# vpc-ccg/circminer

Measured on AMD Instinct MI355X. Metric: paired reads/sec (whole node), hg38 k=20, 2x150 bp; circ_report bit-exact, higher is better.
Workload: dtype int32/u8 (chain scores f64)

## Files before the change

circminer_amd/csrc/cm_hot.hip:

```cpp
#include <chrono>
#include <hip/hip_runtime.h>
#include <rocprim/device/device_radix_sort.hpp>

#include <algorithm>
#include <atomic>
#include <cstdarg>
#include <cstdio>
#include <cstdlib>
#include <cstring>
#include <string>
#include <functional>
#include <thread>
#include <vector>

#include "circminer_hot.h"
#include "cm_core.h"
#include "cm_aos.h"
#include "cm_index_build.h"

using cmc::Core;
using cmc::KCore;

namespace {

constexpr int MAX_SLOTS = 16;
constexpr uint32_t TILE_PAIRS = 1u << 20;
constexpr uint32_t TILE_PAIRS_MAX = 1u << 21;
constexpr int BLK = 256;
constexpr int BLK_CHAIN = 64;
#include "cm_dp_engine.h"

enum ProfClass { PC_NONE = -1, PC_SEED = 0, PC_CHAIN = 1, PC_PAIR = 2, PC_SCAN = 3, PC_HEAVY = 4, PC_ORDER = 5, PC_CHAIN_HEAVY = 6, PC_PREFETCH = 7, PC_COUNT = 8 };
enum Counter {
    CN_PROBES = 0 , CN_PAIR_ROUNDS = 3, CN_RERUN = 4 ,
    CN_FALL = 5, CN_FALL_2ND = 6,
    CN_CD_LANE = 8, CN_CD_PHASE = 13, CN_CD_WAVE = 16, CN_CD_EVENTS = 20, CN_CD_LEVELS = 21, CN_CD_PROBLEMS = 22, CN_CD_PASSES = 23, CN_CD_CELLS = 24,
    CN_HP_ATTEMPT = 8, CN_HP_STRIDE = 8, CN_HP_UNPAIRED = 24, CN_HP_CHAINS = 25, CN_HP_SEQ_TASKS = 26, CN_HP_EARLY = 27, CN_HP_EARLY_FIRST = 28,
    CN_WORDS = 32
};
static_assert(CN_CD_CELLS < CN_WORDS && CN_HP_EARLY_FIRST < CN_WORDS && CN_HP_ATTEMPT + CN_HP_STRIDE + 5 < CN_HP_UNPAIRED, "d_counters has CN_WORDS words");
enum Pin {
    PIN_COLLECT_N = 0, PIN_COLLECT_ERR = 1,
    PIN_DEV_ERR = 0,
    PIN_POOL_ERR = 2,
    PIN_HEAVY_LOAD = 4,
    PIN_CELLS = 8,
    PIN_RERUN_N = 12, PIN_FALL_N = 14,
    PIN_WORDS = 16
};
constexpr size_t PIN_BYTES = PIN_WORDS * sizeof(unsigned long long);
static_assert(PIN_BYTES == 128 && PIN_FALL_N + 1 < PIN_WORDS && PIN_CELLS + 3 < PIN_RERUN_N, "the landing zone has 16 words");
struct ReadsDev {
    const uint8_t *seq1, *seq2;
    const uint64_t *off1, *off2;
};

__global__ void __launch_bounds__(BLK) k_seed(KCore kc, ReadsDev rd, const uint8_t *active, uint64_t pair0, uint32_t n_tile, int S,
                                              uint32_t *sstart, uint32_t *scnt, uint32_t *sraw, unsigned long long *counters) {
    const Core c = cmc::to_core(kc);
    __shared__ unsigned int sh[3];
    if (threadIdx.x < 3) sh[threadIdx.x] = 0;
    __syncthreads();
    const uint64_t q = (uint64_t)blockIdx.x * BLK + threadIdx.x;
    const uint64_t total = (uint64_t)n_tile * 4u * (uint64_t)S;
    if (q < total) {
        const uint32_t s = (uint32_t)(q % (uint64_t)S);
        const uint64_t r = q / (uint64_t)S;
        const int orient = (int)(r & 1u), mate = (int)((r >> 1) & 1u);
        const uint64_t p = pair0 + (r >> 2);
        uint32_t st = 0, cn = 0, rw = 0;
        if (active[p]) {
            const uint64_t o0 = mate ? rd.off2[p] : rd.off1[p], o1 = mate ? rd.off2[p + 1] : rd.off1[p + 1];
            const int len = (int)(o1 - o0);
            const int k = c.P.kmer;
            if ((int)(s + 1) * k <= len) {
                const cmc::Read R{(cmc::g_u8)((mate ? rd.seq2 : rd.seq1) + o0), len, orient};
                const cmc::Probe pr = cmc::seed_probe(c, R.view(), (int)s * k);
                st = pr.start;
                rw = pr.raw;
                cn = (pr.raw > (uint32_t)c.P.seed_lim) ? 0u : pr.raw;
                atomicAdd(&sh[0], 1u);
                atomicAdd(&sh[1], pr.touches);
                atomicAdd(&sh[2], cn);
            }
        }
        sstart[q] = st;
        scnt[q] = cn;
        sraw[q] = rw;
    }
    __syncthreads();
    if (threadIdx.x < 3 && sh[threadIdx.x]) atomicAdd(&counters[CN_PROBES + threadIdx.x], (unsigned long long)sh[threadIdx.x]);
}

constexpr int SCAN_T = 256;
constexpr int SCAN_ELEMS = 1024;
__global__ void __launch_bounds__(SCAN_T) k_scan_a(const uint32_t *scnt, int S, uint32_t n, unsigned long long *out, unsigned long long *bsum,
                                                   unsigned int *bmax) {
    __shared__ unsigned long long sh[SCAN_T];
    __shared__ unsigned int shmax;
    const uint32_t base = blockIdx.x * SCAN_ELEMS;
    unsigned long long run = 0;
    unsigned int my_max = 0;
    if (threadIdx.x == 0) shmax = 0;
#pragma unroll
    for (int k = 0; k < SCAN_ELEMS / SCAN_T; ++k) {
        const uint32_t r = base + k * SCAN_T + threadIdx.x;
        uint32_t c = 0;
        if (r < n)
            for (int s = 0; s < S; ++s) c += scnt[(uint64_t)r * S + s];
        my_max = c > my_max ? c : my_max;
        sh[threadIdx.x] = c;
        __syncthreads();
        for (int d = 1; d < SCAN_T; d <<= 1) {
            const unsigned long long x = (threadIdx.x >= (unsigned)d) ? sh[threadIdx.x - d] : 0ull;
            __syncthreads();
            sh[threadIdx.x] += x;
            __syncthreads();
        }
        if (r < n) out[r] = run + sh[threadIdx.x] - c;
        run += sh[SCAN_T - 1];
        __syncthreads();
    }
    atomicMax(&shmax, my_max);
    __syncthreads();
    if (threadIdx.x == 0) {
        bsum[blockIdx.x] = run;
        bmax[blockIdx.x] = shmax;
    }
}
template <class T, bool WITH_MAX>
__global__ void __launch_bounds__(1024) k_scan_mid(T *bsum, uint32_t nb, T *total, const unsigned int *bmax) {
    __shared__ T part[1024];
    __shared__ unsigned int gmax;
    const uint32_t t = threadIdx.x;
    const uint32_t chunk = (nb + 1023u) / 1024u;
    const uint32_t a = t * chunk, b = (a + chunk < nb) ? a + chunk : nb;
    T s = 0;
    unsigned int m = 0;
    if (WITH_MAX && t == 0) gmax = 0;
    if constexpr (WITH_MAX) __syncthreads();
    for (uint32_t i = a; i < b; ++i) {
        s += bsum[i];
        if constexpr (WITH_MAX) m = bmax[i] > m ? bmax[i] : m;
    }
    if constexpr (WITH_MAX) atomicMax(&gmax, m);
    part[t] = s;
    __syncthreads();
    for (uint32_t d = 1; d < 1024; d <<= 1) {
        const T v = (t >= d) ? part[t - d] : (T)0;
        __syncthreads();
        part[t] += v;
        __syncthreads();
    }
    T run = t ? part[t - 1] : (T)0;
    for (uint32_t i = a; i < b; ++i) {
        const T x = bsum[i];
        bsum[i] = run;
        run += x;
    }
    if (WITH_MAX && t == 1023) {
        total[0] = part[1023];
        total[1] = gmax;
    }
}
__global__ void __launch_bounds__(SCAN_T) k_scan_c(unsigned long long *out, const unsigned long long *bsum, uint32_t n) {
    const uint32_t i = blockIdx.x * SCAN_T + threadIdx.x;
    if (i < n) out[i] += bsum[i / SCAN_ELEMS];
}

__device__ inline int pack_resid(int left, int right) {
    left = left < 0 ? 0 : (left > 255 ? 255 : left);
    right = right < 0 ? 0 : (right > 255 ? 255 : right);
    return left | (right << 8);
}
#ifndef CM_CHAIN_WAVES
#define CM_CHAIN_WAVES 5
#endif
__global__ void __launch_bounds__(BLK_CHAIN, CM_CHAIN_WAVES) k_chain(KCore kc, ReadsDev rd, const uint8_t *active, uint64_t pair0, uint32_t r0, uint32_t r1, int S,
                                                     const uint32_t *sstart, const uint32_t *scnt, const uint32_t *sraw,
                                                     const unsigned long long *celloff, unsigned long long cellbase, double *dp_score,
                                                     int32_t *dp_prev, uint8_t *pool, unsigned long long pool_bytes,
                                                     unsigned long long *pool_cursor, cm_chain *chains, int32_t *nchain, int32_t *high, int *err,
                                                     uint16_t *resid, const uint32_t *perm, const unsigned int *perm_lo, const unsigned int *perm_hi) {
    uint32_t r = r0 + blockIdx.x * BLK_CHAIN + threadIdx.x;
    if (perm) {
        r += *perm_lo;
        if (r >= *perm_hi) return;
        r = perm[r];
    } else if (r >= r1) return;
// ... 2 lines not shown
    int n = 0, hh = 0, rs = 0;
    if (active[p]) {
        const int mate = (int)((r >> 1) & 1u);
        const uint64_t o0 = mate ? rd.off2[p] : rd.off1[p], o1 = mate ? rd.off2[p + 1] : rd.off1[p + 1];
        const int len = (int)(o1 - o0);
        uint32_t st[cmc::MAX_SEEDS], cn[cmc::MAX_SEEDS];
        for (int s = 0; s < S; ++s) {
            st[s] = sstart[(uint64_t)r * S + s];
            cn[s] = scnt[(uint64_t)r * S + s];
            if (sraw[(uint64_t)r * S + s] > 0 && cn[s] == 0) ++hh;
        }
        cmc::ChainWork w;
        w.dp_score = (CM_G double *)(dp_score + (celloff[r] - cellbase));
        w.dp_prev = (CM_G int32_t *)(dp_prev + (celloff[r] - cellbase));
        w.pool = (CM_G uint8_t *)pool;
        w.pool_bytes = pool_bytes;
        w.pool_cursor = (CM_G unsigned long long *)pool_cursor;
        w.err = (cmc::g_err)err;
        n = cmc::chain_kbest(c, len, S, st, cn, w, (CM_G cm_chain *)(chains + (uint64_t)r * CM_BESTCHAINLIM));
        if (n > 0) {
            const cm_chain &b = chains[(uint64_t)r * CM_BESTCHAINLIM];
            rs = pack_resid(b.qpos[0], len - (b.qpos[b.chain_len - 1] + c.P.kmer));
        }
    }
    nchain[r] = n;
    high[r] = hh;
    resid[r] = (uint16_t)rs;
}

struct RetryArgs {
    uint32_t *pair_err;
    uint32_t *list;
    unsigned int *count;
    cmc::MemoSpill *spill;
    int spill_cap;
    int first;
};

template <bool FIRST>
__device__ __forceinline__ void pair_kernel(const KCore &kc, const ReadsDev &rd, uint64_t pair0, uint32_t n_tile, const cm_chain *chains, const int32_t *nchain,
                                            const int32_t *high, cm_mapped_read *state, uint8_t *active, int32_t *cat, int is_last,
                                            int *err, unsigned long long *counters, int str_cap, unsigned long long *lane_clk,
                                            const uint32_t *perm, const unsigned int *n_light, unsigned int *next_chunk,
                                            const RetryArgs &ra) {
    const unsigned long long clk0 = lane_clk ? wall_clock64() : 0ull;
    extern __shared__ uint32_t lds_words[];
#if defined(CM_DIAG)
    __shared__ unsigned long long tick_w[65];
    cmc::Tick tick;
    for (int i = 0; i < 32; ++i) tick.acc[i] = 0;
    tick.last = wall_clock64();
    tick.w = (CM_L unsigned long long *)tick_w;
    tick.wave_on = 1;
    for (int i = threadIdx.x; i < 65; i += BLK_PAIR) tick_w[i] = i == 0 ? tick.last : 0ull;
    __syncthreads();
    cmc::DpMem sm = lane_dp_mem((CM_S uint8_t *)lds_words, threadIdx.x, str_cap, (cmc::g_err)err, &tick);
#else
    cmc::DpMem sm = lane_dp_mem((CM_S uint8_t *)lds_words, threadIdx.x, str_cap, (cmc::g_err)err);
#endif
    if (ra.spill) {
        sm.spill = (cmc::g_spill)(ra.spill + ((size_t)blockIdx.x * BLK_PAIR + threadIdx.x) * (size_t)ra.spill_cap);
        sm.spill_cap = ra.spill_cap;
    }
    const Core c = cmc::to_core(kc);
    const uint32_t n_l = *n_light;
    auto take = [&]() { return (uint32_t)__shfl((int)(threadIdx.x == 0 ? atomicAdd(next_chunk, 1u) : 0u), 0); };
    for (uint32_t chunk = take(); (uint64_t)chunk * BLK_PAIR < n_l; chunk = take()) {
    const uint32_t slot = chunk * BLK_PAIR + threadIdx.x;
    if (slot >= n_l) continue;
    const unsigned long long it0 = lane_clk ? wall_clock64() : 0ull;
    const uint32_t t = perm[slot];
    const uint64_t p = pair0 + t;
    const uint64_t a0 = rd.off1[p], a1 = rd.off1[p + 1], b0 = rd.off2[p], b1 = rd.off2[p + 1];
    cmc::ChainSet sets[4];
    int hh[4];
    for (int x = 0; x < 4; ++x) {
        const uint64_t r = (uint64_t)t * 4 + x;
        sets[x].ch = (cmc::g_chain)(chains + r * CM_BESTCHAINLIM);
        sets[x].n = nchain[r];
        hh[x] = high[r];
    }
    cm_mapped_read mr = state[p];
#if defined(CM_AB_GLOBAL_ERR)
    int *perr = err;
#else
    int *perr = FIRST ? (int *)(ra.pair_err + t) : err;
    sm.err = (cmc::g_err)perr;
#endif
    const int st = cmc::process_read(c, sm, (cmc::g_u8)(rd.seq1 + a0), (int)(a1 - a0), (cmc::g_u8)(rd.seq2 + b0), (int)(b1 - b0), sets, hh, mr, (cmc::g_err)perr);
    bool keep = true;
    if (FIRST) {
        if (__hip_atomic_load(ra.pair_err + t, __ATOMIC_RELAXED, __HIP_MEMORY_SCOPE_AGENT) != 0u) {
            ra.list[atomicAdd(ra.count, 1u)] = t;
            active[pair0 + t] = 1;
            keep = false;
        }
    } else ra.pair_err[t] = 0u;
    if (keep) {
        uint8_t act = 1;
        cmc::finish_round(c, st, is_last, (int)(a1 - a0), (int)(b1 - b0), mr, act);
        state[p] = mr;
        active[p] = act;
        cat[p] = st;
    }
    {
        const unsigned long long m = __ballot(1), mk = __ballot(keep);
        if ((threadIdx.x & 63) == (unsigned)__ffsll((long long)m) - 1 && mk) {
            atomicAdd(&counters[CN_PAIR_ROUNDS], (unsigned long long)__popcll(mk));
            if (!FIRST) atomicAdd(&counters[CN_RERUN], (unsigned long long)__popcll(mk));
        }
    }
#if defined(CM_DIAG)
    CM_TICK(sm, 13);
    if (lane_clk) {
        for (int i = 0; i < 15; ++i) lane_clk[p * 16 + i] = tick.acc[i];
        lane_clk[p * 16 + 15] = wall_clock64() - clk0;
        const unsigned long long m = __ballot(1);
        if ((threadIdx.x & 63) == (unsigned)__ffsll((long long)m) - 1) {
            unsigned long long *wr = lane_clk + (unsigned long long)n_tile * 16 + (unsigned long long)blockIdx.x * 64;
            for (int i = 0; i < 64; ++i) wr[i] = tick_w[1 + i];
        }
    }
#else
    if (lane_clk) lane_clk[slot] = ((wall_clock64() - it0) & 0xFFFFFFFFull) | ((unsigned long long)t << 32);
#endif
    }
}


__global__ void __launch_bounds__(BLK_PAIR, CM_PAIR_WAVES) k_pair(KCore kc, ReadsDev rd, uint64_t pair0, uint32_t n_tile, const cm_chain *chains, const int32_t *nchain,
                                                   const int32_t *high, cm_mapped_read *state, uint8_t *active, int32_t *cat, int is_last,
                                                   int *err, unsigned long long *counters, int str_cap, unsigned long long *lane_clk,
                                                   const uint32_t *perm, const unsigned int *n_light, unsigned int *next_chunk,
                                                   RetryArgs ra) {
    pair_kernel<true>(kc, rd, pair0, n_tile, chains, nchain, high, state, active, cat, is_last, err, counters, str_cap, lane_clk, perm, n_light, next_chunk, ra);
}
__global__ void __launch_bounds__(BLK_PAIR, CM_PAIR_WAVES) k_pair_rerun(KCore kc, ReadsDev rd, uint64_t pair0, uint32_t n_tile, const cm_chain *chains,
                                                         const int32_t *nchain, const int32_t *high, cm_mapped_read *state, uint8_t *active, int32_t *cat,
                                                         int is_last, int *err, unsigned long long *counters, int str_cap,
                                                         unsigned long long *lane_clk, const uint32_t *perm, const unsigned int *n_light,
                                                         unsigned int *next_chunk, RetryArgs ra) {
    pair_kernel<false>(kc, rd, pair0, n_tile, chains, nchain, high, state, active, cat, is_last, err, counters, str_cap, lane_clk, perm, n_light, next_chunk, ra);
}

template <class T> __device__ inline T wave_excl_scan(T v, int lane, T &total) {
    T x = v;
    for (int o = 1; o < 64; o <<= 1) {
        const T y = __shfl_up(x, o);
        if (lane >= o) x += y;
    }
    total = __shfl(x, 63);
    return x - v;
}
struct HeavyChainCtx {
#if defined(CM_CHAIN_DIAG)
    unsigned long long *tk;
#endif
    const Core *c;
    CM_L const uint32_t *LP;
    CM_L const uint32_t *NB;
    CM_L const uint32_t *IM;
    const uint32_t *base, *cnt;
    int kc, seq_len;
    CM_G double *dps;
    CM_G int32_t *dpp;
};
__device__ inline uint32_t heavy_im_word(uint32_t base_s, uint32_t s) { return 2u * ((base_s >> 6) + s); }
__host__ __device__ inline uint32_t heavy_im_words(uint32_t ncell, uint32_t kc) { return 2u * ((ncell >> 6) + kc + 1u); }
__device__ inline uint32_t heavy_cell(const HeavyChainCtx &h, int ii, uint32_t i, CM_G cmc::Event *ev, double &out_score, int32_t &out_prev,
                                     double &e0, double &e1) {
    const Core &c = *h.c;
    const int kmer = c.P.kmer;
    const uint32_t read_remain = (uint32_t)(h.seq_len - ii * kmer - kmer);
    const int32_t cur_info = (int32_t)h.LP[h.base[ii] + i];
    const uint32_t seg_start = (uint32_t)cur_info, seg_end = (uint32_t)cur_info + kmer - 1;
    uint32_t max_lpos_lim = cmc::MAXUB, max_exon_end = 0;
    int ol = -1;
    double my_score = (double)kmer;
    int32_t my_prev = -1;
    uint32_t n = 0;
    const uint32_t cell = h.base[ii] + i;
    const bool near = (h.NB[cell >> 5] >> (cell & 31)) & 1u;
    uint2 parked = make_uint2(0u, 0u);
    int parked_ol = -1;
    if (near) {
        parked = *(CM_G const uint2 *)(h.dps + cell);
        parked_ol = h.dpp[cell];
    }
#if defined(CM_CHAIN_DIAG)
    if (!ev) h.tk[3] += 1;
#define CD_T0 const unsigned long long cd_t = wall_clock64()
#define CD_ADD(k) h.tk[k] += wall_clock64() - cd_t
#else
#define CD_T0
#define CD_ADD(k)
#endif
    for (int jj = ii + 1; jj < h.kc; ++jj) {
        const uint32_t pcn = h.cnt[jj];
        if (pcn == 0) continue;
        CM_L const uint32_t *pp = h.LP + h.base[jj];
        CM_L const uint32_t *im = h.IM + heavy_im_word(h.base[jj], (uint32_t)jj);
        uint32_t lo = 0, hi = pcn;
        {
            CD_T0;
            while (lo < hi) {
                const uint32_t mid = (lo + hi) >> 1;
                if ((int32_t)pp[mid] <= cur_info) lo = mid + 1;
                else hi = mid;
            }
            CD_ADD(0);
        }
        if (lo >= pcn) continue;
        if (cur_info + c.P.max_intron < (int32_t)pp[lo]) continue;
        if (max_lpos_lim == cmc::MAXUB) {
            CD_T0;
            if (near) {
                max_lpos_lim = parked.x;
                max_exon_end = parked.y;
                ol = parked_ol;
            } else {
                max_exon_end = 0;
                ol = -1;
                max_lpos_lim = seg_start + read_remain + (uint32_t)c.P.max_ed;
            }
            CD_ADD(1);
        }
        const int distr = (jj - ii) * kmer - kmer;
        CD_T0;
        for (uint32_t j = lo; j < pcn && pp[j] <= max_lpos_lim; ++j) {
#if defined(CM_CHAIN_DIAG)
            if (!ev) h.tk[4] += 1;
#endif
            const uint32_t pinfo = pp[j];
            int genome_dist, distt, trans_dist;
            if (max_exon_end == 0 || (pinfo + kmer - 1) <= max_exon_end) genome_dist = (int)(pinfo - seg_end - 1);
            else genome_dist = cmc::INF_I;
            if (cmc::cabs(genome_dist - distr) <= c.P.max_ed) distt = genome_dist;
            else if (cmc::check_junction(c, seg_start, pinfo, ol, kmer, distr, trans_dist)) distt = trans_dist;
            else continue;
            const int maxd = distr < distt ? distt : distr, mind = distr < distt ? distr : distt;
            const double beta = 0.1 * (double)(maxd - mind);
            const double alpha = 2e4 * (double)kmer;
            const double prev_score = ((im[j >> 5] >> (j & 31)) & 1u) ? h.dps[h.base[jj] + j] : (double)kmer;
            const double t1 = prev_score + alpha;
            const double temp_score = t1 - beta;
            if (temp_score > my_score) {
                my_score = temp_score;
                my_prev = (int32_t)(((uint32_t)jj << 16) | j);
                if (ev) {
                    ev[n].score = temp_score;
                    ev[n].cell = ((uint32_t)ii << 16) | i;
                }
                if (n == 0) e0 = temp_score;
                else if (n == 1) e1 = temp_score;
                ++n;
            }
        }
        CD_ADD(2);
    }
    out_score = my_score;
    out_prev = my_prev;
    return n;
}

struct HeavyBackTrack {
    uint32_t base[cmc::MAX_SEEDS + 1];
    uint32_t cand[CM_BESTCHAINLIM + 2];
    uint16_t cidx[CM_BESTCHAINLIM][CM_MAX_CHAIN_FRAGS];
    uint8_t cbl[CM_BESTCHAINLIM][CM_MAX_CHAIN_FRAGS];
    uint8_t clen[CM_BESTCHAINLIM + 2];
    uint8_t emit[CM_BESTCHAINLIM + 2];
    uint32_t rep[CM_BESTCHAINLIM * (CM_MAX_CHAIN_FRAGS - 1)];
};

#ifndef CM_CHEAVY_WAVES
#define CM_CHEAVY_WAVES 3
#endif
__global__ void __launch_bounds__(64, CM_CHEAVY_WAVES) k_chain_heavy(KCore kc_, ReadsDev rd, uint64_t pair0, int S, const uint32_t *sstart, const uint32_t *scnt,
                                                    const unsigned long long *celloff, double *dp_score, int32_t *dp_prev, uint8_t *pool,
                                                    unsigned long long pool_bytes, unsigned long long *pool_cursor, cm_chain *chains, int32_t *nchain,
                                                    int *err, uint16_t *resid, const uint32_t *perm, const unsigned int *n_perm, unsigned int *next_problem,
                                                    unsigned long long *counters) {
    extern __shared__ uint32_t lds_words[];
    CM_L uint32_t *LP = (CM_L uint32_t *)lds_words;
    __shared__ HeavyBackTrack BT;
    const int lane = threadIdx.x;
    const Core c = cmc::to_core(kc_);
    const int kmer = c.P.kmer;
    const uint32_t max_best = (uint32_t)c.P.max_chain_len;
    const unsigned int n_heavy = *n_perm;
    auto take = [&]() { return (unsigned int)__shfl((int)(lane == 0 ? atomicAdd(next_problem, 1u) : 0u), 0); };
    for (unsigned int hidx = take(); hidx < n_heavy; hidx = take()) {
        const uint32_t r = perm[hidx];
        const uint64_t p = pair0 + (r >> 2);
        const int mate = (int)((r >> 1) & 1u);
        const int len = (int)(mate ? rd.off2[p + 1] - rd.off2[p] : rd.off1[p + 1] - rd.off1[p]);
#if defined(CM_CHAIN_DIAG)
        const unsigned long long dg0 = wall_clock64();
#endif
        uint32_t st[cmc::MAX_SEEDS], cn[cmc::MAX_SEEDS], base[cmc::MAX_SEEDS + 1];
        int kc = S;
        for (int s = 0; s < S; ++s) {
            st[s] = sstart[(uint64_t)r * S + s];
            cn[s] = scnt[(uint64_t)r * S + s];
        }
        while (kc >= 1 && cn[kc - 1] == 0) --kc;
        base[0] = 0;
        for (int s = 0; s < kc; ++s) base[s + 1] = base[s] + cn[s];
        const uint32_t ncell = base[kc];
        CM_G double *dps = (CM_G double *)(dp_score + celloff[r]);
        CM_G int32_t *dpp = (CM_G int32_t *)(dp_prev + celloff[r]);
        CM_L uint32_t *NB = LP + ncell;
        CM_L uint16_t *Q = (CM_L uint16_t *)(NB + 2 * ((ncell + 63) >> 6));
        CM_L uint32_t *IM = (CM_L uint32_t *)(Q + 320);
        const bool by_entry = c.entry_near != nullptr;
        for (int s = 0; s < kc; ++s)
            for (uint32_t i = lane; i < cn[s]; i += 64) {
                const uint32_t e = st[s] + i;
                uint32_t v = c.X.pos[e];
                if (by_entry && s < kc - 1) v |= (uint32_t)((c.entry_near[e >> 6] >> (e & 63)) & 1ull) << 31;
                LP[base[s] + i] = v;
            }
        for (uint32_t x = lane; x < heavy_im_words(ncell, (uint32_t)kc); x += 64) IM[x] = 0u;
        __threadfence_block();
        __syncthreads();
        {
            const uint32_t n_pre = kc >= 1 ? base[kc - 1] : 0u;
            const unsigned long long lt = (1ull << lane) - 1ull;
            uint32_t qn = 0;
            auto look_up = [&](uint32_t cnt) {
                if ((uint32_t)lane < cnt) {
                    const uint32_t x = Q[lane];
                    int ii = 0;
                    for (int s = 1; s < kc; ++s) ii += x >= base[s] ? 1 : 0;
                    const uint32_t read_remain = (uint32_t)(len - ii * kmer - kmer);
                    uint32_t mx = 0;
                    int ol = -1;
                    const uint32_t lim = cmc::upper_bound_lookup(c, LP[x], (uint32_t)kmer, read_remain, mx, ol);
                    *(CM_G uint2 *)(dps + x) = make_uint2(lim, mx);
                    dpp[x] = ol;
                }
            };
            for (uint32_t x0 = 0; x0 < n_pre; x0 += 256) {
                bool nr[4];
#pragma unroll
                for (int u = 0; u < 4; ++u) {
                    const uint32_t x = x0 + 64 * u + lane;
                    if (by_entry) {
                        nr[u] = x < n_pre && (LP[x] >> 31);
                        if (nr[u]) LP[x] &= 0x7fffffffu;
                    } else nr[u] = x < n_pre && cmc::bit_at(c.A.near_border_bits, c.A.n_bits, LP[x]);
                }
#pragma unroll
                for (int u = 0; u < 4; ++u) {
                    const uint32_t xb = x0 + 64 * u;
                    if (xb >= n_pre) break;
                    const unsigned long long m = __ballot(nr[u]);
                    if (lane == 0) NB[xb >> 5] = (uint32_t)m;
                    if (lane == 32) NB[(xb >> 5) + 1] = (uint32_t)(m >> 32);
                    if (nr[u]) Q[qn + __popcll(m & lt)] = (uint16_t)(xb + lane);
                    qn += (uint32_t)__popcll(m);
                }
                __syncthreads();
                while (qn >= 64) {
                    look_up(64);
                    uint16_t keep[4];
#pragma unroll
                    for (int u = 0; u < 4; ++u) keep[u] = 64u * u + (uint32_t)lane < qn - 64 ? Q[64 + 64 * u + lane] : (uint16_t)0;
                    __syncthreads();
#pragma unroll
                    for (int u = 0; u < 4; ++u)
                        if (64u * u + (uint32_t)lane < qn - 64) Q[64 * u + lane] = keep[u];
                    qn -= 64;
                    __syncthreads();
                }
            }
            if (qn) look_up(qn);
        }
        __threadfence_block();
        __syncthreads();
#if defined(CM_CHAIN_DIAG)
        const unsigned long long dg1 = wall_clock64();
#endif
#if defined(CM_CHAIN_DIAG)
        unsigned long long tk[5] = {0, 0, 0, 0, 0};
        unsigned long long wv[4] = {0, 0, 0, 0};
        HeavyChainCtx H{tk, &c, LP, NB, IM, base, cn, kc, len, dps, dpp};
#else
        HeavyChainCtx H{&c, LP, NB, IM, base, cn, kc, len, dps, dpp};
#endif
        CM_G cmc::Event *ev = nullptr;
        uint32_t n_ev = 0, cap_ev = 0;
        bool lost = false;
        for (int ii = kc - 2; ii >= 0; --ii) {
            for (uint32_t i0 = 0; i0 < cn[ii]; i0 += 64) {
                const uint32_t i = i0 + lane;
                const bool on = i < cn[ii];
                double sc = 0, e0 = 0, e1 = 0;
                int32_t pv = -1;
#if defined(CM_CHAIN_DIAG)
                const unsigned long long w0 = wall_clock64();
#endif
                const uint32_t mine = on ? heavy_cell(H, ii, i, (CM_G cmc::Event *)nullptr, sc, pv, e0, e1) : 0u;
#if defined(CM_CHAIN_DIAG)
                const unsigned long long w1 = wall_clock64();
#endif
                {
                    const unsigned long long m = __ballot(mine > 0u);
                    const uint32_t w = heavy_im_word(base[ii], (uint32_t)ii) + (i0 >> 5);
                    if (lane == 0) IM[w] = (uint32_t)m;
                    if (lane == 32) IM[w + 1] = (uint32_t)(m >> 32);
                }
                uint32_t total;
                const uint32_t off = wave_excl_scan(mine, lane, total);
                if (n_ev + total > cap_ev && !lost) {
                    uint32_t ncap = cap_ev ? cap_ev : 256u;
                    while (ncap < n_ev + total) ncap *= 4u;
                    const unsigned long long bytes = (unsigned long long)ncap * sizeof(cmc::Event);
                    unsigned long long o = 0;
                    if (lane == 0) o = atomicAdd(pool_cursor, bytes);
                    o = ((unsigned long long)__shfl((unsigned int)(o >> 32), 0) << 32) | (unsigned long long)__shfl((unsigned int)o, 0);
                    if (o + bytes > pool_bytes) {
                        lost = true;
                        if (lane == 0) atomicOr(err, cmc::ERR_POOL);
                    } else {
                        CM_G cmc::Event *ne = (CM_G cmc::Event *)((CM_G uint8_t *)pool + o);
                        for (uint32_t q = lane; q < n_ev; q += 64) ne[q] = ev[q];
                        ev = ne;
                        cap_ev = ncap;
                    }
                }
                if (on && mine) {
                    if (!lost) {
                        CM_G cmc::Event *dst = ev + n_ev + off;
                        if (mine <= 2) {
                            dst[0].score = e0;
                            dst[0].cell = ((uint32_t)ii << 16) | i;
                            if (mine == 2) {
                                dst[1].score = e1;
                                dst[1].cell = ((uint32_t)ii << 16) | i;
                            }
                        } else heavy_cell(H, ii, i, dst, sc, pv, e0, e1);
                    }
                    dps[base[ii] + i] = sc;
                    dpp[base[ii] + i] = pv;
                }
                if (!lost) n_ev += total;
#if defined(CM_CHAIN_DIAG)
                const unsigned long long w3 = wall_clock64();
                wv[0] += w1 - w0;
                wv[2] += w3 - w1;
#endif
            }
#if defined(CM_CHAIN_DIAG)
            const unsigned long long w4 = wall_clock64();
#endif
            __threadfence_block();
            __syncthreads();
#if defined(CM_CHAIN_DIAG)
            wv[3] += wall_clock64() - w4;
#endif
        }
#if defined(CM_CHAIN_DIAG)
        for (int k = 0; k < 5; ++k) atomicAdd(&counters[CN_CD_LANE + k], tk[k]);
        if (lane == 0)
            for (int k = 0; k < 4; ++k) atomicAdd(&counters[CN_CD_WAVE + k], wv[k]);
#endif
        CM_G cm_chain *out = (CM_G cm_chain *)(chains + (uint64_t)r * CM_BESTCHAINLIM);
        uint32_t best_count = 0;
        int first_q0 = 0, first_qlast = 0;
        if (lane <= kc) BT.base[lane] = base[lane];
        __threadfence_block();
        __syncthreads();
#if defined(CM_CHAIN_DIAG)
        const unsigned long long dg2 = wall_clock64();
#endif
        if (n_ev > 0) {
            double best_score = -1.0;
            for (uint32_t q = lane; q < n_ev; q += 64) best_score = ev[q].score > best_score ? ev[q].score : best_score;
            for (int o = 32; o >= 1; o >>= 1) {
                const double u = __shfl_xor(best_score, o);
                best_score = u > best_score ? u : best_score;
            }
            double cur = best_score;
            bool have = true;
            uint32_t n_rep = 0;
#if defined(CM_CHAIN_DIAG)
            unsigned long long dg_levels = 0;
#endif
            while (have && best_count < max_best) {
#if defined(CM_CHAIN_DIAG)
                ++dg_levels;
#endif
                uint32_t n_c = 0;
                double nxt = -1.0;
                bool hv = false;
                for (uint32_t q0 = 0; q0 < n_ev; q0 += 64) {
                    const uint32_t q = q0 + lane;
                    const double v = q < n_ev ? ev[q].score : 0.0;
                    const bool hit = q < n_ev && v == cur;
                    if (q < n_ev && v < cur && (!hv || v > nxt)) {
                        nxt = v;
                        hv = true;
                    }
                    const unsigned long long m = __ballot(hit);
                    if (m && n_c < max_best) {
                        const uint32_t rank = n_c + (uint32_t)__popcll(m & ((1ull << lane) - 1ull));
                        if (hit && rank < max_best) BT.cand[rank] = ev[q].cell;
                        n_c += (uint32_t)__popcll(m);
                        if (n_c > max_best) n_c = max_best;
                    }
                }
                for (int o = 32; o >= 1; o >>= 1) {
                    const double u = __shfl_xor(nxt, o);
                    const int uh = __shfl_xor((int)hv, o);
                    if (uh && (!hv || u > nxt)) {
                        nxt = u;
                        hv = true;
                    }
                }
                __syncthreads();
                if ((uint32_t)lane < n_c) {
                    const uint32_t cell = BT.cand[lane];
                    uint32_t bl = cell >> 16, bi = cell & 0xffffu, n = 0;
                    while (true) {
                        const uint32_t x = BT.base[bl] + bi;
                        BT.cidx[lane][n] = (uint16_t)x;
                        BT.cbl[lane][n] = (uint8_t)bl;
                        ++n;
                        const bool improved = (IM[heavy_im_word(BT.base[bl], bl) + (bi >> 5)] >> (bi & 31)) & 1u;
                        const int32_t pv = improved ? dpp[x] : -1;
                        if (pv < 0 || n >= (uint32_t)CM_MAX_CHAIN_FRAGS) break;
                        bl = (uint32_t)pv >> 16;
                        bi = (uint32_t)pv & 0xffffu;
                    }
                    BT.clen[lane] = (uint8_t)n;
                }
                __syncthreads();
                const uint32_t first = best_count;
                uint32_t n_emit = 0;
                for (uint32_t a = 0; a < n_c && best_count < max_best; ++a) {
                    if (cur < best_score) {
                        const uint32_t spos = LP[BT.cidx[a][0]];
                        bool mine = false;
                        for (uint32_t x = lane; x < n_rep; x += 64) mine = mine || BT.rep[x] == spos;
                        if (__ballot(mine) != 0ull) continue;
                    }
                    const uint32_t cl = BT.clen[a];
                    if (lane == 0) BT.emit[n_emit] = (uint8_t)a;
                    if ((uint32_t)lane >= 1u && (uint32_t)lane < cl) BT.rep[n_rep + lane - 1] = LP[BT.cidx[a][lane]];
                    if (best_count == 0) {
                        first_q0 = (int)BT.cbl[a][0] * kmer;
                        first_qlast = (int)BT.cbl[a][cl - 1] * kmer;
                    }
                    n_rep += cl - 1;
                    ++n_emit;
                    ++best_count;
                    __syncthreads();
                }
                __syncthreads();
                for (uint32_t x = lane; x < n_emit * (uint32_t)CM_MAX_CHAIN_FRAGS; x += 64) {
                    const uint32_t k = x / (uint32_t)CM_MAX_CHAIN_FRAGS, f = x % (uint32_t)CM_MAX_CHAIN_FRAGS;
                    const uint32_t a = BT.emit[k];
                    if (f < BT.clen[a]) {
                        CM_G cm_chain &ch = out[first + k];
                        ch.rpos[f] = LP[BT.cidx[a][f]];
                        ch.qpos[f] = (int32_t)BT.cbl[a][f] * kmer;
                    }
                }
                if ((uint32_t)lane < n_emit) {
                    CM_G cm_chain &ch = out[first + lane];
                    ch.score = (float)cur;
                    ch.chain_len = BT.clen[BT.emit[lane]];
                }
                __syncthreads();
                have = hv;
                cur = nxt;
            }
#if defined(CM_CHAIN_DIAG)
            if (lane == 0) {
                atomicAdd(&counters[CN_CD_EVENTS], (unsigned long long)n_ev);
                atomicAdd(&counters[CN_CD_LEVELS], dg_levels);
                atomicAdd(&counters[CN_CD_PROBLEMS], 1ull);
                atomicAdd(&counters[CN_CD_PASSES], dg_levels * (unsigned long long)((n_ev + 63) / 64));
                atomicAdd(&counters[CN_CD_CELLS], (unsigned long long)ncell);
            }
#endif
        }
        if (best_count == 0) {
            for (int ii = kc - 1; ii >= 0; --ii)
                for (uint32_t i = 0; i < cn[ii]; ++i) {
                    if (best_count >= max_best) break;
                    if (best_count == 0) first_q0 = first_qlast = ii * kmer;
                    if (lane == 0) {
                        CM_G cm_chain &ch = out[best_count];
                        ch.rpos[0] = LP[base[ii] + i];
                        ch.qpos[0] = ii * kmer;
                        ch.score = (float)(double)kmer;
                        ch.chain_len = 1;
                    }
                    ++best_count;
                }
        }
        __threadfence_block();
        __syncthreads();
        if (lane == 0) {
            nchain[r] = (int32_t)best_count;
            int rs = 0;
            if (best_count > 0) rs = pack_resid(first_q0, len - (first_qlast + kmer));
            resid[r] = (uint16_t)rs;
#if defined(CM_CHAIN_DIAG)
            const unsigned long long dg3 = wall_clock64();
            atomicAdd(&counters[CN_CD_PHASE + 0], dg1 - dg0);
            atomicAdd(&counters[CN_CD_PHASE + 1], dg2 - dg1);
            atomicAdd(&counters[CN_CD_PHASE + 2], dg3 - dg2);
#endif
        }
        __syncthreads();
    }
}

constexpr int HEAVY_COST = 6;
constexpr int N_BUCKETS = 7;
constexpr int HEAVY_CLS = 15;
__device__ inline int pair_class(const Core &c, const cm_chain *chains, const uint16_t *resid4, const int32_t *nchain,
                                 const uint8_t *active, uint64_t pair0, uint32_t t, int heavy_cost, int *sub) {
    const uint64_t p = pair0 + t;
    if (sub) *sub = 0;
    if (!active[p]) return -2;
    const int32_t *nc = nchain + 4 * (uint64_t)t;
    const int a = nc[0], b = nc[1], cc = nc[2], d = nc[3];
    if ((a + b) > 0 && (cc + d) > 0 && (a * d + cc * b + a + b + cc + d) > heavy_cost) {
        if (sub) {
            const int cost = a * d + cc * b + a + b + cc + d;
            const int lv = cost <= 12 ? 0 : cost <= 16 ? 1 : cost <= 24 ? 2 : cost <= 32 ? 3 : cost <= 48 ? 4 : cost <= 64 ? 5 : cost <= 96 ? 6 : cost <= 128 ? 7
                           : cost <= 192 ? 8 : cost <= 256 ? 9 : cost <= 384 ? 10 : cost <= 512 ? 11 : cost <= 768 ? 12 : 13;
            *sub = lv << 4;
        }
        return HEAVY_CLS;
    }
    const uint16_t *q = resid4 + 4 * (uint64_t)t;
    int resid = 0;
    for (int x = 0; x < 4; ++x) resid += (q[x] & 0xff) + (q[x] >> 8);
    if (sub) {
        const bool main0 = a > 0 && d > 0;
        const uint16_t f = q[main0 ? 0 : 2], bk = q[main0 ? 3 : 1];
        *sub = ((f & 0xff) ? 1 : 0) | ((f >> 8) ? 2 : 0) | ((bk & 0xff) ? 4 : 0) | ((bk >> 8) ? 8 : 0);
        int mx = f & 0xff;
        mx = (f >> 8) > mx ? (f >> 8) : mx;
        mx = (bk & 0xff) > mx ? (bk & 0xff) : mx;
        mx = (bk >> 8) > mx ? (bk >> 8) : mx;
        const int lv = mx < 5 ? 0 : mx < 10 ? 1 : mx < 15 ? 2 : mx < 20 ? 3 : mx < 25 ? 4 : mx < 30 ? 5 : mx < 40 ? 6 : mx < 50 ? 7 : mx < 60 ? 8 : mx < 70 ? 9
                       : mx < 80 ? 10 : mx < 90 ? 11 : mx < 100 ? 12 : mx < 115 ? 13 : mx < 130 ? 14 : 15;
        *sub |= lv << 4;
    }
    const int bucket = resid < 25 ? 0 : resid < 50 ? 1 : resid < 100 ? 2 : resid < 150 ? 3 : resid < 200 ? 4 : resid < 300 ? 5 : 6;
    bool genic = false;
    for (int x = 0; x < 4 && !genic; ++x) {
        if (nc[x] <= 0) continue;
        genic = cmc::overlap(c, chains[((uint64_t)t * 4 + x) * CM_BESTCHAINLIM].rpos[0]) >= 0;
    }
    return (genic ? N_BUCKETS : 0) + bucket;
}
constexpr int CHAIN_LIGHT_CLS = 12;
constexpr int CLS_T = 1024;
constexpr int CLS_W = 256;
constexpr int CLS_REP = CLS_T / CLS_W;
constexpr int N_CLS = 16;
constexpr int CTR_SUM = 16, CTR_BASE = 32, CTR_WORDS = 64;
constexpr int CTR_NEXT = 48;
constexpr int CTR_RETRY = 50;
constexpr int CTR_CHAIN_NEXT = 48;
static_assert(CTR_CHAIN_NEXT >= CTR_BASE + N_CLS && CTR_CHAIN_NEXT < CTR_WORDS && CTR_NEXT >= CTR_BASE + N_CLS && CTR_RETRY + 1 < CTR_WORDS, "spare words");
constexpr unsigned HEAVY_GRID_MAX = 4096;
constexpr int RETRY_GRID = 8;
constexpr int RETRY_SPILL = 2040;
__device__ inline void block_class_ranks(int k, unsigned int (*wcnt)[N_CLS], unsigned int &rank_in_wave, int lane, int wave) {
    rank_in_wave = 0;
#pragma unroll
    for (int c = 0; c < N_CLS; ++c) {
        const unsigned long long m = __ballot(k == c);
        if (lane == 0) wcnt[wave][c] = (unsigned int)__popcll(m);
        if (k == c) rank_in_wave = (unsigned int)__popcll(m & ((1ull << lane) - 1ull));
    }
}
constexpr int HEAVY_COST_WIDE = 16;
constexpr unsigned long long HEAVY_LOAD = 16;
__global__ void __launch_bounds__(BLK) k_pair_cost(const int32_t *nchain, const uint8_t *active, uint64_t pair0, uint32_t n_tile, int base_cost,
                                                  unsigned long long *sum) {
    __shared__ unsigned long long sh[BLK / 64];
    const uint32_t t = blockIdx.x * BLK + threadIdx.x;
    unsigned long long v = 0;
    if (t < n_tile && active[pair0 + t]) {
        const int32_t *nc = nchain + 4 * (uint64_t)t;
        const int a = nc[0], b = nc[1], cc = nc[2], d = nc[3];
        const int cost = a * d + cc * b + a + b + cc + d;
        if ((a + b) > 0 && (cc + d) > 0 && cost > base_cost) v = (unsigned long long)cost;
    }
    for (int o = 32; o >= 1; o >>= 1) v += __shfl_xor(v, o);
    if ((threadIdx.x & 63) == 0) sh[threadIdx.x >> 6] = v;
    __syncthreads();
    if (threadIdx.x == 0) {
        unsigned long long s2 = 0;
        for (int w = 0; w < BLK / 64; ++w) s2 += sh[w];
        if (s2) atomicAdd(sum, s2);
    }
}
__global__ void __launch_bounds__(BLK) k_pair_cls(KCore kc, const cm_chain *chains, const uint16_t *resid, const int32_t *nchain,
                                                 const uint8_t *active, uint64_t pair0, uint32_t n_tile, int8_t *cls, int32_t *cat, int heavy_cost,
                                                 int8_t *cls_sub, int8_t *cls_sub2, uint8_t *act_out, const unsigned long long *heavy_load) {
    const uint32_t t = blockIdx.x * BLK + threadIdx.x;
    if (t >= n_tile) return;
    const Core c = cmc::to_core(kc);
    if (heavy_load && *heavy_load > HEAVY_LOAD * (unsigned long long)n_tile) heavy_cost = HEAVY_COST_WIDE;
    int sub = 0;
    const int k = pair_class(c, chains, resid, nchain, active, pair0, t, heavy_cost, &sub);
    cls[t] = (int8_t)k;
    cls_sub[t] = (int8_t)(k < 0 ? -2 : (k == HEAVY_CLS ? 0 : (sub & 15)));
    cls_sub2[t] = (int8_t)(k < 0 ? -2 : (sub >> 4));
    if (k == -2) {
        cat[pair0 + t] = -1;
        act_out[pair0 + t] = 0;
    }
}
__global__ void __launch_bounds__(BLK) k_chain_cls(const uint32_t *scnt, const uint32_t *sraw, int S, uint32_t n_prob, int8_t *cls, int32_t *high,
                                                  unsigned long long light_w, unsigned int light_cells, int32_t *nchain, uint16_t *resid,
                                                  const uint8_t *active, uint64_t pair0) {
    const uint32_t r = blockIdx.x * BLK + threadIdx.x;
    if (r >= n_prob) return;
    if (!active[pair0 + (r >> 2)]) {
        high[r] = 0;
        if (nchain) {
            nchain[r] = 0;
            resid[r] = 0;
        }
        cls[r] = -2;
        return;
    }
    unsigned long long w = 0, suffix = 0;
    int hh = 0;
    for (int s = S - 1; s >= 0; --s) {
        const unsigned long long c = scnt[(uint64_t)r * S + s];
        w += c * suffix;
        suffix += c;
        if (sraw[(uint64_t)r * S + s] > 0 && c == 0) ++hh;
    }
    high[r] = hh;
    if (suffix == 0 && nchain) {
        nchain[r] = 0;
        resid[r] = 0;
    }
    const bool light = w <= light_w && suffix <= light_cells;
    const unsigned int n = (unsigned int)suffix;
    cls[r] = (int8_t)(suffix == 0 ? -2
                      : light ? (n <= 3 ? 0 : n <= 6 ? 1 : n <= 7 ? 2 : n <= 9 ? 3 : n <= 12 ? 4 : n <= 16 ? 5 : n <= 24 ? 6 : n <= 32 ? 7 : n <= 48 ? 8 : n <= 64 ? 9
                                 : n <= 96 ? 10 : 11)
                      : w <= 4096 ? 12 : w <= 65536 ? 13 : w <= 1048576 ? 14 : 15);
}
__global__ void __launch_bounds__(BLK) k_chain_apply(uint32_t n_prob, const int8_t *cls, const int32_t *thigh, int32_t *high, int32_t *nchain, uint16_t *resid) {
    const uint32_t r = blockIdx.x * BLK + threadIdx.x;
    if (r >= n_prob) return;
    high[r] = thigh[r];
    if (cls[r] == -2) {
        nchain[r] = 0;
        resid[r] = 0;
    }
}
__global__ void __launch_bounds__(CLS_W) k_cls_hist(const int8_t *cls, uint32_t n, unsigned int *blk_cnt, uint32_t nb, const uint32_t *order,
                                                    const unsigned int *n_order) {
    __shared__ unsigned int wcnt[CLS_T / 64][N_CLS];
    const uint32_t lim = n_order ? (*n_order < n || order ? *n_order : n) : n;
// ... 2671 lines not shown
```

Before: 28.89 million.

## Prefetch next heavy-chain problem, batch predecessor loads, keep event log in registers

The heavy-chain kernel now fetches the next problem's index, seed headers and offsets while the current problem is being chained, and broadcasts them with readfirstlane/readlane instead of per-thread loads. The predecessor scan loads the first candidate score for four seed groups up front so the global loads overlap. For small event logs, the backtrack level selection keeps events in registers and gathers several score levels per batch instead of rescanning the global event log once per level. The max score is tracked during DP rather than rescanned. In exchange there is more register pressure, more control complexity, and a risk of speculative loads that go unused.

```diff
diff --git a/circminer_amd/csrc/cm_hot.hip b/circminer_amd/csrc/cm_hot.hip
--- a/circminer_amd/csrc/cm_hot.hip
+++ b/circminer_amd/csrc/cm_hot.hip
@@ -35,6 +35,7 @@
     CN_PROBES = 0 , CN_PAIR_ROUNDS = 3, CN_RERUN = 4 ,
     CN_FALL = 5, CN_FALL_2ND = 6,
     CN_CD_LANE = 8, CN_CD_PHASE = 13, CN_CD_WAVE = 16, CN_CD_EVENTS = 20, CN_CD_LEVELS = 21, CN_CD_PROBLEMS = 22, CN_CD_PASSES = 23, CN_CD_CELLS = 24,
+    CN_CD_REGLOG = 25, CN_CD_BATCHES = 26, CN_CD_PRE_USED = 27, CN_CD_PRE_UNUSED = 28,
     CN_HP_ATTEMPT = 8, CN_HP_STRIDE = 8, CN_HP_UNPAIRED = 24, CN_HP_CHAINS = 25, CN_HP_SEQ_TASKS = 26, CN_HP_EARLY = 27, CN_HP_EARLY_FIRST = 28,
     CN_WORDS = 32
 };
@@ -343,6 +344,9 @@
     total = __shfl(x, 63);
     return x - v;
 }
+#ifndef CM_CHEAVY_LOG_REGS
+#define CM_CHEAVY_LOG_REGS 4
+#endif
 struct HeavyChainCtx {
 #if defined(CM_CHAIN_DIAG)
     unsigned long long *tk;
@@ -386,11 +390,27 @@
 #define CD_T0
 #define CD_ADD(k)
 #endif
-    for (int jj = ii + 1; jj < h.kc; ++jj) {
+    const uint32_t own_lim = seg_start + read_remain + (uint32_t)c.P.max_ed;
+    for (int j0 = ii + 1; j0 < h.kc; j0 += 4) {
+    uint32_t g_lo[4];
+    double g_sc[4];
+    bool g_ok[4];
+#if defined(CM_CHAIN_DIAG)
+    bool g_ld[4];
+#endif
+#pragma unroll
+    for (int g = 0; g < 4; ++g) {
+        const int jj = j0 + g;
+        g_ok[g] = false;
+        g_lo[g] = 0;
+        g_sc[g] = (double)kmer;
+#if defined(CM_CHAIN_DIAG)
+        g_ld[g] = false;
+#endif
+        if (jj >= h.kc) continue;
         const uint32_t pcn = h.cnt[jj];
         if (pcn == 0) continue;
         CM_L const uint32_t *pp = h.LP + h.base[jj];
-        CM_L const uint32_t *im = h.IM + heavy_im_word(h.base[jj], (uint32_t)jj);
         uint32_t lo = 0, hi = pcn;
         {
             CD_T0;
@@ -402,7 +422,28 @@
             CD_ADD(0);
         }
         if (lo >= pcn) continue;
-        if (cur_info + c.P.max_intron < (int32_t)pp[lo]) continue;
+        const uint32_t first = pp[lo];
+        if (cur_info + c.P.max_intron < (int32_t)first) continue;
+        g_ok[g] = true;
+        g_lo[g] = lo;
+        if ((near || first <= own_lim) && ((h.IM[heavy_im_word(h.base[jj], (uint32_t)jj) + (lo >> 5)] >> (lo & 31)) & 1u)) {
+            g_sc[g] = h.dps[h.base[jj] + lo];
+#if defined(CM_CHAIN_DIAG)
+            g_ld[g] = true;
+#endif
+        }
+    }
+#pragma unroll
+    for (int g = 0; g < 4; ++g) {
+        if (!g_ok[g]) continue;
+        const int jj = j0 + g;
+        const uint32_t pcn = h.cnt[jj];
+        CM_L const uint32_t *pp = h.LP + h.base[jj];
+        CM_L const uint32_t *im = h.IM + heavy_im_word(h.base[jj], (uint32_t)jj);
+        const uint32_t lo = g_lo[g];
+#if defined(CM_CHAIN_DIAG)
+        bool g_used = false;
+#endif
         if (max_lpos_lim == cmc::MAXUB) {
             CD_T0;
             if (near) {
@@ -432,7 +473,10 @@
             const int maxd = distr < distt ? distt : distr, mind = distr < distt ? distr : distt;
             const double beta = 0.1 * (double)(maxd - mind);
             const double alpha = 2e4 * (double)kmer;
-            const double prev_score = ((im[j >> 5] >> (j & 31)) & 1u) ? h.dps[h.base[jj] + j] : (double)kmer;
+            const double prev_score = j == lo ? g_sc[g] : ((im[j >> 5] >> (j & 31)) & 1u) ? h.dps[h.base[jj] + j] : (double)kmer;
+#if defined(CM_CHAIN_DIAG)
+            if (j == lo) g_used = true;
+#endif
             const double t1 = prev_score + alpha;
             const double temp_score = t1 - beta;
             if (temp_score > my_score) {
@@ -442,12 +486,16 @@
                     ev[n].score = temp_score;
                     ev[n].cell = ((uint32_t)ii << 16) | i;
                 }
-                if (n == 0) e0 = temp_score;
-                else if (n == 1) e1 = temp_score;
+                e1 = n == 1 ? temp_score : e1;
+                e0 = n == 0 ? temp_score : e0;
                 ++n;
             }
         }
         CD_ADD(2);
+#if defined(CM_CHAIN_DIAG)
+        if (!ev && g_ld[g]) h.tk[g_used ? 5 : 6] += 1;
+#endif
+    }
     }
     out_score = my_score;
     out_prev = my_prev;
@@ -480,27 +528,45 @@
     const int kmer = c.P.kmer;
     const uint32_t max_best = (uint32_t)c.P.max_chain_len;
     const unsigned int n_heavy = *n_perm;
-    auto take = [&]() { return (unsigned int)__shfl((int)(lane == 0 ? atomicAdd(next_problem, 1u) : 0u), 0); };
-    for (unsigned int hidx = take(); hidx < n_heavy; hidx = take()) {
-        const uint32_t r = perm[hidx];
-        const uint64_t p = pair0 + (r >> 2);
-        const int mate = (int)((r >> 1) & 1u);
-        const int len = (int)(mate ? rd.off2[p + 1] - rd.off2[p] : rd.off1[p + 1] - rd.off1[p]);
+    auto take_raw = [&]() { return lane == 0 ? atomicAdd(next_problem, 1u) : 0u; };
+    uint32_t nx_r = 0, nx_st = 0, nx_cn = 0;
+    unsigned long long nx_coff = 0, nx_o0 = 0, nx_o1 = 0;
+    auto ask_header = [&](uint32_t rr) {
+        nx_st = lane < S ? sstart[(uint64_t)rr * S + lane] : 0u;
+        nx_cn = lane < S ? scnt[(uint64_t)rr * S + lane] : 0u;
+        nx_coff = celloff[rr];
+        const uint64_t pp = pair0 + (rr >> 2);
+        const uint64_t *of = ((rr >> 1) & 1u) ? rd.off2 : rd.off1;
+        nx_o0 = of[pp];
+        nx_o1 = of[pp + 1];
+    };
+    unsigned int hidx = (unsigned int)__builtin_amdgcn_readfirstlane((int)take_raw());
+    if (hidx < n_heavy) {
+        nx_r = perm[hidx];
+        ask_header(nx_r);
+    }
+    while (hidx < n_heavy) {
+        const uint32_t r = (uint32_t)__builtin_amdgcn_readfirstlane((int)nx_r);
+        const unsigned int nx_raw = take_raw();
+        const int len = __builtin_amdgcn_readfirstlane((int)(nx_o1 - nx_o0));
+        const unsigned long long coff = ((unsigned long long)(uint32_t)__builtin_amdgcn_readfirstlane((int)(nx_coff >> 32)) << 32) |
+                                        (unsigned long long)(uint32_t)__builtin_amdgcn_readfirstlane((int)nx_coff);
 #if defined(CM_CHAIN_DIAG)
         const unsigned long long dg0 = wall_clock64();
 #endif
         uint32_t st[cmc::MAX_SEEDS], cn[cmc::MAX_SEEDS], base[cmc::MAX_SEEDS + 1];
         int kc = S;
-        for (int s = 0; s < S; ++s) {
-            st[s] = sstart[(uint64_t)r * S + s];
-            cn[s] = scnt[(uint64_t)r * S + s];
+#pragma unroll
+        for (int s = 0; s < cmc::MAX_SEEDS; ++s) {
+            st[s] = (uint32_t)__builtin_amdgcn_readlane((int)nx_st, s);
+            cn[s] = (uint32_t)__builtin_amdgcn_readlane((int)nx_cn, s);
         }
         while (kc >= 1 && cn[kc - 1] == 0) --kc;
         base[0] = 0;
         for (int s = 0; s < kc; ++s) base[s + 1] = base[s] + cn[s];
         const uint32_t ncell = base[kc];
-        CM_G double *dps = (CM_G double *)(dp_score + celloff[r]);
-        CM_G int32_t *dpp = (CM_G int32_t *)(dp_prev + celloff[r]);
+        CM_G double *dps = (CM_G double *)(dp_score + coff);
+        CM_G int32_t *dpp = (CM_G int32_t *)(dp_prev + coff);
         CM_L uint32_t *NB = LP + ncell;
         CM_L uint16_t *Q = (CM_L uint16_t *)(NB + 2 * ((ncell + 63) >> 6));
         CM_L uint32_t *IM = (CM_L uint32_t *)(Q + 320);
@@ -574,15 +640,18 @@
         const unsigned long long dg1 = wall_clock64();
 #endif
 #if defined(CM_CHAIN_DIAG)
-        unsigned long long tk[5] = {0, 0, 0, 0, 0};
+        unsigned long long tk[7] = {0, 0, 0, 0, 0, 0, 0};
         unsigned long long wv[4] = {0, 0, 0, 0};
         HeavyChainCtx H{tk, &c, LP, NB, IM, base, cn, kc, len, dps, dpp};
 #else
         HeavyChainCtx H{&c, LP, NB, IM, base, cn, kc, len, dps, dpp};
 #endif
+        const unsigned int hnext = (unsigned int)__builtin_amdgcn_readfirstlane((int)nx_raw);
+        if (hnext < n_heavy) nx_r = perm[hnext];
         CM_G cmc::Event *ev = nullptr;
         uint32_t n_ev = 0, cap_ev = 0;
         bool lost = false;
+        double lane_best = -1.0;
         for (int ii = kc - 2; ii >= 0; --ii) {
             for (uint32_t i0 = 0; i0 < cn[ii]; i0 += 64) {
                 const uint32_t i = i0 + lane;
@@ -635,6 +704,7 @@
                     }
                     dps[base[ii] + i] = sc;
                     dpp[base[ii] + i] = pv;
+                    lane_best = sc > lane_best ? sc : lane_best;
                 }
                 if (!lost) n_ev += total;
 #if defined(CM_CHAIN_DIAG)
@@ -654,6 +724,8 @@
         }
 #if defined(CM_CHAIN_DIAG)
         for (int k = 0; k < 5; ++k) atomicAdd(&counters[CN_CD_LANE + k], tk[k]);
+        atomicAdd(&counters[CN_CD_PRE_USED], tk[5]);
+        atomicAdd(&counters[CN_CD_PRE_UNUSED], tk[6]);
         if (lane == 0)
             for (int k = 0; k < 4; ++k) atomicAdd(&counters[CN_CD_WAVE + k], wv[k]);
 #endif
@@ -666,49 +738,122 @@
 #if defined(CM_CHAIN_DIAG)
         const unsigned long long dg2 = wall_clock64();
 #endif
+        if (hnext < n_heavy) ask_header((uint32_t)__builtin_amdgcn_readfirstlane((int)nx_r));
         if (n_ev > 0) {
-            double best_score = -1.0;
-            for (uint32_t q = lane; q < n_ev; q += 64) best_score = ev[q].score > best_score ? ev[q].score : best_score;
+            constexpr int LR = CM_CHEAVY_LOG_REGS;
+            constexpr uint32_t CAP = CM_BESTCHAINLIM;
+            const unsigned long long lt = (1ull << lane) - 1ull;
+            double best_score = lane_best;
             for (int o = 32; o >= 1; o >>= 1) {
                 const double u = __shfl_xor(best_score, o);
                 best_score = u > best_score ? u : best_score;
             }
+            const bool in_regs = n_ev <= 64u * (uint32_t)LR;
+            const int n_u = (int)((n_ev + 63u) >> 6);
+            double es[LR];
+            uint32_t ec[LR];
+#pragma unroll
+            for (int u = 0; u < LR; ++u) {
+                es[u] = -1.0;
+                ec[u] = 0u;
+                const uint32_t q = (uint32_t)lane + 64u * (uint32_t)u;
+                if (in_regs && q < n_ev) {
+                    const cmc::Event e = ev[q];
+                    es[u] = e.score;
+                    ec[u] = e.cell;
+                }
+            }
             double cur = best_score;
             bool have = true;
             uint32_t n_rep = 0;
+            int lv_u = 0;
+            unsigned long long lv_done = 0;
+            uint32_t lv_taken = 0;
+            double my_cs = 0.0;
 #if defined(CM_CHAIN_DIAG)
-            unsigned long long dg_levels = 0;
+            unsigned long long dg_levels = 0, dg_passes = 0, dg_batches = 0;
 #endif
             while (have && best_count < max_best) {
+                uint32_t n_c = 0;
 #if defined(CM_CHAIN_DIAG)
-                ++dg_levels;
-#endif
-                uint32_t n_c = 0;
-                double nxt = -1.0;
-                bool hv = false;
-                for (uint32_t q0 = 0; q0 < n_ev; q0 += 64) {
-                    const uint32_t q = q0 + lane;
-                    const double v = q < n_ev ? ev[q].score : 0.0;
-                    const bool hit = q < n_ev && v == cur;
-                    if (q < n_ev && v < cur && (!hv || v > nxt)) {
-                        nxt = v;
-                        hv = true;
+                ++dg_batches;
+#endif
+                if (in_regs) {
+#if defined(CM_CHAIN_DIAG)
+                    if (dg_passes == 0) dg_passes = (unsigned long long)n_u;
+#endif
+                    while (have && n_c < CAP) {
+                        const uint32_t n_c0 = n_c;
+#if defined(CM_CHAIN_DIAG)
+                        if (lv_u == 0 && lv_taken == 0 && lv_done == 0ull) ++dg_levels;
+#endif
+#pragma unroll
+                        for (int u = 0; u < LR; ++u) {
+                            if (u < lv_u || u >= n_u || lv_taken >= max_best || n_c >= CAP) continue;
+                            const bool hit = es[u] == cur && !((lv_done >> lane) & 1ull);
+                            const unsigned long long m = __ballot(hit);
+                            const uint32_t n_m = (uint32_t)__popcll(m);
+                            const uint32_t room = max_best - lv_taken < CAP - n_c ? max_best - lv_taken : CAP - n_c;
+                            const bool tk = hit && (uint32_t)__popcll(m & lt) < room;
+                            if (tk) BT.cand[n_c + (uint32_t)__popcll(m & lt)] = ec[u];
+                            if (n_m > room) {
+                                lv_done |= __ballot(tk);
+                                lv_u = u;
+                                n_c += room;
+                                lv_taken += room;
+                            } else {
+                                lv_done = 0ull;
+                                lv_u = u + 1;
+                                n_c += n_m;
+                                lv_taken += n_m;
+                            }
+                        }
+                        if ((uint32_t)lane >= n_c0 && (uint32_t)lane < n_c) my_cs = cur;
+                        if (lv_taken >= max_best || lv_u >= n_u) {
+                            double nxt = -1.0;
+#pragma unroll
+                            for (int u = 0; u < LR; ++u)
+                                if (es[u] < cur && es[u] > nxt) nxt = es[u];
+                            for (int o = 32; o >= 1; o >>= 1) {
+                                const double v = __shfl_xor(nxt, o);
+                                nxt = v > nxt ? v : nxt;
+                            }
+                            have = nxt >= 0.0;
+                            cur = nxt;
+                            lv_u = 0;
+                            lv_done = 0ull;
+                            lv_taken = 0;
+                        }
                     }
-                    const unsigned long long m = __ballot(hit);
-                    if (m && n_c < max_best) {
-                        const uint32_t rank = n_c + (uint32_t)__popcll(m & ((1ull << lane) - 1ull));
-                        if (hit && rank < max_best) BT.cand[rank] = ev[q].cell;
-                        n_c += (uint32_t)__popcll(m);
-                        if (n_c > max_best) n_c = max_best;
+                } else {
+#if defined(CM_CHAIN_DIAG)
+                    ++dg_levels;
+                    dg_passes += (unsigned long long)n_u;
+#endif
+                    double nxt = -1.0;
+                    for (uint32_t q0 = 0; q0 < n_ev; q0 += 64) {
+                        const uint32_t q = q0 + lane;
+                        cmc::Event e;
+                        e.score = -1.0;
+                        e.cell = 0u;
+                        if (q < n_ev) e = ev[q];
+                        const bool hit = q < n_ev && e.score == cur;
+                        if (q < n_ev && e.score < cur && e.score > nxt) nxt = e.score;
+                        const unsigned long long m = __ballot(hit);
+                        if (m && n_c < max_best) {
+                            const uint32_t rank = n_c + (uint32_t)__popcll(m & lt);
+                            if (hit && rank < max_best) BT.cand[rank] = e.cell;
+                            n_c += (uint32_t)__popcll(m);
+                            if (n_c > max_best) n_c = max_best;
+                        }
                     }
-                }
-                for (int o = 32; o >= 1; o >>= 1) {
-                    const double u = __shfl_xor(nxt, o);
-                    const int uh = __shfl_xor((int)hv, o);
-                    if (uh && (!hv || u > nxt)) {
-                        nxt = u;
-                        hv = true;
+                    for (int o = 32; o >= 1; o >>= 1) {
+                        const double v = __shfl_xor(nxt, o);
+                        nxt = v > nxt ? v : nxt;
                     }
+                    if ((uint32_t)lane < n_c) my_cs = cur;
+                    have = nxt >= 0.0;
+                    cur = nxt;
                 }
                 __syncthreads();
                 if ((uint32_t)lane < n_c) {
@@ -731,7 +876,7 @@
                 const uint32_t first = best_count;
                 uint32_t n_emit = 0;
                 for (uint32_t a = 0; a < n_c && best_count < max_best; ++a) {
-                    if (cur < best_score) {
+                    if (__shfl(my_cs, (int)a) < best_score) {
                         const uint32_t spos = LP[BT.cidx[a][0]];
                         bool mine = false;
                         for (uint32_t x = lane; x < n_rep; x += 64) mine = mine || BT.rep[x] == spos;
@@ -759,22 +904,23 @@
                         ch.qpos[f] = (int32_t)BT.cbl[a][f] * kmer;
                     }
                 }
+                const double cs = __shfl(my_cs, (uint32_t)lane < n_emit ? (int)BT.emit[lane] : 0);
                 if ((uint32_t)lane < n_emit) {
                     CM_G cm_chain &ch = out[first + lane];
-                    ch.score = (float)cur;
+                    ch.score = (float)cs;
                     ch.chain_len = BT.clen[BT.emit[lane]];
                 }
                 __syncthreads();
-                have = hv;
-                cur = nxt;
             }
 #if defined(CM_CHAIN_DIAG)
             if (lane == 0) {
                 atomicAdd(&counters[CN_CD_EVENTS], (unsigned long long)n_ev);
                 atomicAdd(&counters[CN_CD_LEVELS], dg_levels);
                 atomicAdd(&counters[CN_CD_PROBLEMS], 1ull);
-                atomicAdd(&counters[CN_CD_PASSES], dg_levels * (unsigned long long)((n_ev + 63) / 64));
+                atomicAdd(&counters[CN_CD_PASSES], dg_passes);
                 atomicAdd(&counters[CN_CD_CELLS], (unsigned long long)ncell);
+                atomicAdd(&counters[CN_CD_REGLOG], in_regs ? 1ull : 0ull);
+                atomicAdd(&counters[CN_CD_BATCHES], dg_batches);
             }
 #endif
         }
@@ -808,6 +954,7 @@
 #endif
         }
         __syncthreads();
+        hidx = hnext;
     }
 }
 
```

New measurement: 29.73 million (median of 6 runs). +2.9%, better.
